# ginevracoal/robustBNNs

Hardware: AMD Instinct MI355X
Metric: attack-samples/sec (test_pts x posterior_samples x PGD_iters) (higher is better)
Workload: dtype f32 (full-width operands as three f16 pieces: 6 exact f16 MFMA product terms per fp32 product, f32 accumulate)

## Files before the change

### include/robustbnns_hip.h

```cpp
#ifndef ROBUSTBNNS_HIP_H
#define ROBUSTBNNS_HIP_H

#include <stddef.h>
#include <stdint.h>

#ifdef __cplusplus
extern "C" {
#endif

#define RBNN_ABI_VERSION 10
#define RBNN_CPAD 16

typedef enum rbnn_status {
    RBNN_OK = 0,
    RBNN_ERR_NULL = -1,
    RBNN_ERR_SHAPE = -2,
    RBNN_ERR_UNSUPPORTED = -3,
    RBNN_ERR_LAUNCH = -4,
    RBNN_ERR_ALIGN = -5
} rbnn_status;

typedef enum rbnn_activation { RBNN_ACT_RELU = 0, RBNN_ACT_LEAKY = 1, RBNN_ACT_SIGM = 2, RBNN_ACT_TANH = 3 } rbnn_activation;
typedef enum rbnn_arch { RBNN_ARCH_FC = 0, RBNN_ARCH_FC2 = 1 } rbnn_arch;

// ... 49 lines not shown
int rbnn_reduce_samples(const float *P, int32_t n_samples, int32_t n_points, int32_t n_classes,
                        float scale, float *out, int32_t ldo, void *stream);

int rbnn_loss_dlogits(int32_t mode, const float *P, const float *Psum, int32_t ldp, const float *G_up,
                      const int32_t *labels, int32_t n_samples, float inv_S, int32_t n_points,
                      int32_t n_classes, float *dZ, void *stream);

int rbnn_fc_input_grad(const rbnn_posterior *net, const int32_t *sample_idx, int32_t n_samples,
                       int32_t n_points, int32_t chunk, const rbnn_workspace *ws,
                       int32_t *n_slabs_out, void *stream);

int rbnn_sum_slabs(const float *slabs, int32_t n_slabs, int32_t n_points, int32_t d_pad, float scale,
                   float *out, int32_t ldo, void *stream);

int rbnn_sum_slabs_norms(const float *slabs, int32_t n_slabs, int32_t n_points, int32_t d_pad, int32_t in_features, float scale,
                         float *out, int32_t ldo, float *linf, float *l2, void *stream);

int rbnn_pgd_alpha(const float *X0, int32_t ldx, int32_t n_points, int32_t in_features,
                   float *alpha, void *stream);

int rbnn_attack_step(float *X, const float *X0, int32_t ldx, const float *G, int32_t n_slabs,
                     size_t slab_stride, int32_t ldg, const float *alpha, float alpha_scalar,
                     float eps, int32_t project, int32_t n_points, int32_t in_features, void *stream);

int rbnn_eval_metrics(const float *out_orig, const float *out_adv, int32_t ldp, const int32_t *labels,
                      int32_t n_points, int32_t n_classes, int32_t *counts, float *rob, void *stream);

int rbnn_pack_rows4(const float *W, int64_t rows, int32_t cols, float *out, void *stream);

typedef struct rbnn_dev_scale {
    uint32_t absmax_bits;
    int32_t  exp;
    float    scale;
    float    inv_scale;
} rbnn_dev_scale;

int rbnn_input_scales(const float *X, int64_t rows, int32_t cols, int32_t ld, float floor_abs, float mul, float add,
                      float cap, rbnn_dev_scale *out, void *stream);

typedef struct rbnn_conv_posterior {
    int32_t activation;
    int32_t hidden;
    int32_t n_classes;
    int32_t n_stored;
    int32_t in_channels;
    int32_t in_width;
// ... 567 lines not shown
```

### robustbnns_amd/_hip.py

```python
import ctypes as C
import os

import torch

from . import _header
from ._header import HipError

_HERE = os.path.dirname(os.path.abspath(__file__))
LIB_PATH = os.path.join(_HERE, "csrc", "librbnn_hip.so")
HEADER_PATH = os.path.join(os.path.dirname(_HERE), "include", "robustbnns_hip.h")

STRUCTS = {
    "Posterior": "rbnn_posterior", "Workspace": "rbnn_workspace", "WorkspaceSizes": "rbnn_workspace_sizes",
    "ConvPosterior": "rbnn_conv_posterior", "ConvWorkspace": "rbnn_conv_workspace", "ConvWorkspaceSizes": "rbnn_conv_workspace_sizes",
    "PieceImages": "rbnn_triple_images", "SplitImages": "rbnn_triple_images", "TripleImages": "rbnn_triple_images",
    "SplitWorkspace": "rbnn_split_workspace", "SplitWorkspaceSizes": "rbnn_split_workspace_sizes",
    "TripleWorkspace": "rbnn_triple_workspace", "TripleWorkspaceSizes": "rbnn_triple_workspace_sizes",
    "SviGuide": "rbnn_svi_guide", "SviFlatTensor": "rbnn_svi_flat_tensor", "SviTrainNet": "rbnn_svi_train_net", "SviTrainWs": "rbnn_svi_train_ws",
    "NnTrainNet": "rbnn_nn_train_net", "NnTrainWs": "rbnn_nn_train_ws",
    "ConvTrainNet": "rbnn_conv_train_net", "ConvTrainWs": "rbnn_conv_train_ws", "ConvTrainBytes": "rbnn_conv_train_bytes",
    "ConvSviTrainNet": "rbnn_conv_svi_train_net",
    "ConvEnsNet": "rbnn_conv_ens_net", "ConvEnsWs": "rbnn_conv_ens_ws", "ConvEnsBytes": "rbnn_conv_ens_bytes",
    "ConvSviLockstepNet": "rbnn_conv_svi_guides_net", "ConvSviLockstepWs": "rbnn_conv_svi_guides_ws", "ConvSviLockstepBytes": "rbnn_conv_svi_guides_bytes",
    "HmcChain": "rbnn_hmc_chain", "HmcLockstep": "rbnn_hmc_lockstep", "ConvHmcChainsNet": "rbnn_conv_hmc_chains_net", "SviLockstep": "rbnn_svi_multi", "SviLockstepAcc": "rbnn_svi_multi_acc",
# ... 117 lines not shown
        check(self.lib.rbnn_loss_dlogits(mode, ptr(P), ptr(Psum), ldp, ptr(G_up), ptr(labels), S, inv_S, N, Cn,
                                         ptr(dZ), stream_of(P)), "rbnn_loss_dlogits")

    def fc_input_grad(self, net, sidx, S, N, chunk, ws):
        w = self._ws(ws)
        n = C.c_int32(0)
        check(self.lib.rbnn_fc_input_grad(C.byref(net.descriptor()), ptr(sidx), S, N, chunk, C.byref(w), C.byref(n),
                                          stream_of(ws["dZ"])), "rbnn_fc_input_grad")
        return n.value

    def sum_slabs(self, slabs, K, N, Dp, scale, out):
        require_gpu(slabs, "slabs")
        check(self.lib.rbnn_sum_slabs(ptr(slabs), K, N, Dp, scale, ptr(out), out.stride(0), stream_of(slabs)), "rbnn_sum_slabs")

    def sum_slabs_norms(self, slabs, K, N, Dp, D, scale, out, linf, l2):
        require_gpu(slabs, "slabs")
        check(self.lib.rbnn_sum_slabs_norms(ptr(slabs), K, N, Dp, D, scale, ptr(out), out.stride(0), ptr(linf), ptr(l2),
                                            stream_of(slabs)), "rbnn_sum_slabs_norms")

    def pgd_alpha(self, X0, D, alpha):
        require_gpu(X0, "X0")
        check(self.lib.rbnn_pgd_alpha(ptr(X0), X0.stride(0), X0.shape[0], D, ptr(alpha), stream_of(X0)), "rbnn_pgd_alpha")

    def attack_step(self, X, X0, G, K, slab_stride, ldg, alpha, alpha_scalar, eps, project, D):
        require_gpu(X, "X")
        check(self.lib.rbnn_attack_step(ptr(X), ptr(X0), X.stride(0), ptr(G), K, slab_stride, ldg, ptr(alpha),
                                        alpha_scalar, eps, int(project), X.shape[0], D, stream_of(X)), "rbnn_attack_step")

    def eval_metrics(self, A, B, labels, Cn, counts, rob):
        require_gpu(A, "outputs")
        check(self.lib.rbnn_eval_metrics(ptr(A), ptr(B), A.stride(0), ptr(labels), A.shape[0], Cn, ptr(counts), ptr(rob),
                                         stream_of(A)), "rbnn_eval_metrics")

    def pack_rows4(self, W, out):
        require_gpu(W, "W")
        cols = W.shape[-1]
        check(self.lib.rbnn_pack_rows4(ptr(W), W.numel() // cols, cols, ptr(out), stream_of(W)), "rbnn_pack_rows4")

    def input_scales(self, X, cols, floor_abs, mul, add, cap, out):
        require_gpu(X, "X")
        check(self.lib.rbnn_input_scales(ptr(X), X.shape[0], cols, X.stride(0), floor_abs, mul, add, cap, ptr(out), stream_of(X)),
              "rbnn_input_scales")
        return out

    def _rows_image(self, name, src, cols, scale_exp, out, ld_dst, dev_scale):
        require_gpu(src, "src")
        ld_src = src.shape[-1]
        check(getattr(self.lib, name)(ptr(src), src.numel() // ld_src, cols, ld_src, scale_exp, ptr(dev_scale), ptr(out), ld_dst, stream_of(src)), name)
# ... 231 lines not shown
```

### robustbnns_amd/csrc/rbnn_kernels.hip

```cpp
#include "rbnn_common.hpp"
#include <stdlib.h>

namespace {

struct FwdArgs {
    const float* X;   long long x_sample_stride;  int ldx;  int N;
    const float* W;   long long w_sample_stride;  int ldw;  int KT;
    const float* b;
    const float* W2;  const float* b2;            int C;    int H;
    const int* sidx;  int S;   int NT;
    float* P;  uint32_t* mask;  float* dact;  float* hid;  int out_kind;
};

template <int ACT, int WH, int HTW, int WN, int NTW, bool LAYER2>
__global__ void __launch_bounds__(64 * WH * WN, (HTW * NTW > 16 ? 2 : (WH * WN) / 2)) fc_forward_kernel(const FwdArgs a) {
    constexpr int BH = WH * HTW * 16, BN = WN * NTW * 16;
    constexpr int TILE = (BH + BN) * 16;
    constexpr bool BITMASK = (ACT == RBNN_ACT_RELU || ACT == RBNN_ACT_LEAKY);
    constexpr int NW = WH * WN;
    static_assert(NW == 4 || NW == 8, "4 or 8 waves per block");
    static_assert(HTW % 2 == 0 && HTW <= 8, "a wave's h range is whole 32-bit mask words, at most 4");
    static_assert(WH * BN * 16 <= 2 * TILE, "the Z^T reduction scratch aliases the tile buffers");
    __shared__ __attribute__((aligned(16))) float lds[2 * TILE];
    float* const zred = lds;
// ... 424 lines not shown
        f32x4 sum = *(const f32x4*)(slabs + off);
        for (int k = 1; k < K; ++k) sum += *(const f32x4*)(slabs + k * slab_stride + off);
        sum = sum * scale;
        *(f32x4*)(out + (long long)n * ldo + c) = sum;
#pragma unroll
        for (int r = 0; r < 4; ++r)
            if (c + r < D) { m = fmaxf(m, fabsf(sum[r])); ss = fmaf(sum[r], sum[r], ss); }
    }
#pragma unroll
    for (int o = 32; o > 0; o >>= 1) { m = fmaxf(m, __shfl_xor(m, o)); ss += __shfl_xor(ss, o); }
    if (lane == 0) { linf[n] = m; l2[n] = sqrtf(ss); }
}

__global__ void pgd_alpha_kernel(const float* __restrict__ X0, int ldx, int N, int D, float* __restrict__ alpha) {
    const int n = blockIdx.x * (blockDim.x >> 6) + (threadIdx.x >> 6), lane = threadIdx.x & 63;
    if (n >= N) return;
    float m = -INFINITY;
    for (int d = lane; d < D; d += 64) m = fmaxf(m, X0[(long long)n * ldx + d]);
#pragma unroll
    for (int o = 32; o > 0; o >>= 1) m = fmaxf(m, __shfl_xor(m, o));
    if (lane == 0) alpha[n] = 2.f / m;
}

__global__ void attack_step_kernel(float* __restrict__ X, const float* __restrict__ X0, int ldx,
                                   const float* __restrict__ G, int K, long long slab_stride, int ldg,
                                   const float* __restrict__ alpha, float alpha_scalar, float eps, int project,
                                   int N, int D) {
    const long long i = (long long)blockIdx.x * blockDim.x + threadIdx.x;
    if (i >= (long long)N * D) return;
    const long long n = i / D;
    const int d = (int)(i % D);
    float g = G[n * ldg + d];
    for (int k = 1; k < K; ++k) g += G[k * slab_stride + n * ldg + d];
    const float sgn = (g > 0.f) ? 1.f : ((g < 0.f) ? -1.f : 0.f);
    const float step = alpha ? alpha[n] : alpha_scalar;
    const float x = X[n * ldx + d];
    float pert = x + step * sgn;
    if (project) {
        const float x0 = X0[n * ldx + d];
        const float eta = fminf(fmaxf(pert - x0, -eps), eps);
        pert = x0 + eta;
    }
    X[n * ldx + d] = fminf(fmaxf(pert, 0.f), 1.f);
}

__global__ void attack_step4_kernel(float* __restrict__ X, const float* __restrict__ X0, int ldx,
                                    const float* __restrict__ G, int K, long long slab_stride, int ldg,
                                    const float* __restrict__ alpha, float alpha_scalar, float eps, int project,
                                    int N, int D4) {
    const long long i = (long long)blockIdx.x * blockDim.x + threadIdx.x;
    if (i >= (long long)N * D4) return;
    const long long n = i / D4;
    const int d = 4 * (int)(i % D4);
    f32x4 g = *(const f32x4*)(G + n * ldg + d);
    for (int k = 1; k < K; ++k) g += *(const f32x4*)(G + k * slab_stride + n * ldg + d);
    const float step = alpha ? alpha[n] : alpha_scalar;
    const f32x4 x = *(const f32x4*)(X + n * ldx + d);
    f32x4 x0 = x, out;
    if (project) x0 = *(const f32x4*)(X0 + n * ldx + d);
#pragma unroll
    for (int r = 0; r < 4; ++r) {
        const float sgn = (g[r] > 0.f) ? 1.f : ((g[r] < 0.f) ? -1.f : 0.f);
        float pert = x[r] + step * sgn;
        if (project) pert = x0[r] + fminf(fmaxf(pert - x0[r], -eps), eps);
        out[r] = fminf(fmaxf(pert, 0.f), 1.f);
    }
    *(f32x4*)(X + n * ldx + d) = out;
}

__global__ void eval_metrics_kernel(const float* __restrict__ A, const float* __restrict__ B, int ldp,
                                    const int* __restrict__ labels, int N, int C, int* __restrict__ counts,
                                    float* __restrict__ rob) {
    const int n = blockIdx.x * blockDim.x + threadIdx.x;
    int ok_a = 0, ok_b = 0;
    if (n < N) {
        float ma = -INFINITY, mb = -INFINITY;
        int ia = 0, ib = 0;
        for (int c = 0; c < C; ++c) {
            const float a = A[(long long)n * ldp + c], b = B[(long long)n * ldp + c];
            if (a > ma) { ma = a; ia = c; }
            if (b > mb) { mb = b; ib = c; }
        }
        float da = 0.f, db = 0.f;
        for (int c = 0; c < C; ++c) { da += expf(A[(long long)n * ldp + c] - ma); db += expf(B[(long long)n * ldp + c] - mb); }
        float diff = 0.f;
        for (int c = 0; c < C; ++c)
            diff = fmaxf(diff, fabsf(expf(A[(long long)n * ldp + c] - ma) / da - expf(B[(long long)n * ldp + c] - mb) / db));
        rob[n] = 1.f - diff;
        ok_a = (ia == labels[n]);
        ok_b = (ib == labels[n]);
// ... 261 lines not shown
    const long long total4 = (long long)N * d_pad / 4;
    hipLaunchKernelGGL(sum_slabs_kernel, dim3((unsigned)((total4 + 255) / 256)), dim3(256), 0, (hipStream_t)stream,
                       slabs, K, (long long)N * d_pad, total4, d_pad / 4, scale, out, ldo);
    return launch_status();
}

int rbnn_sum_slabs_norms(const float* slabs, int32_t K, int32_t N, int32_t d_pad, int32_t D, float scale, float* out, int32_t ldo,
                         float* linf, float* l2, void* stream) {
    if (!slabs || !out || !linf || !l2) return RBNN_ERR_NULL;
    if (K < 1 || N < 1 || d_pad < 4 || (d_pad & 3) || ldo < d_pad || (ldo & 3) || D < 1 || D > d_pad) return RBNN_ERR_SHAPE;
    if (!aligned16(slabs) || !aligned16(out)) return RBNN_ERR_ALIGN;
    hipLaunchKernelGGL(sum_slabs_norms_kernel, dim3((unsigned)((N + 3) / 4)), dim3(256), 0, (hipStream_t)stream,
                       slabs, K, (long long)N * d_pad, N, d_pad, D, scale, out, ldo, linf, l2);
    return launch_status();
}

int rbnn_pgd_alpha(const float* X0, int32_t ldx, int32_t N, int32_t D, float* alpha, void* stream) {
    if (!X0 || !alpha) return RBNN_ERR_NULL;
    if (N < 1 || D < 1 || ldx < D) return RBNN_ERR_SHAPE;
    hipLaunchKernelGGL(pgd_alpha_kernel, dim3((N + 3) / 4), dim3(256), 0, (hipStream_t)stream, X0, ldx, N, D, alpha);
    return launch_status();
}

int rbnn_attack_step(float* X, const float* X0, int32_t ldx, const float* G, int32_t K, size_t slab_stride, int32_t ldg,
                     const float* alpha, float alpha_scalar, float eps, int32_t project, int32_t N, int32_t D, void* stream) {
    if (!X || !G || (project && !X0)) return RBNN_ERR_NULL;
    if (N < 1 || D < 1 || ldx < D || ldg < D || K < 1) return RBNN_ERR_SHAPE;
    if (!(D & 3) && !(ldx & 3) && !(ldg & 3) && !(slab_stride & 3) && aligned16(X) && aligned16(G) && (!project || aligned16(X0))) {
        const long long total4 = (long long)N * (D / 4);
        hipLaunchKernelGGL(attack_step4_kernel, dim3((unsigned)((total4 + 255) / 256)), dim3(256), 0, (hipStream_t)stream,
                           X, X0, ldx, G, K, (long long)slab_stride, ldg, alpha, alpha_scalar, eps, project, N, D / 4);
        return launch_status();
    }
    const long long total = (long long)N * D;
    hipLaunchKernelGGL(attack_step_kernel, dim3((unsigned)((total + 255) / 256)), dim3(256), 0, (hipStream_t)stream,
                       X, X0, ldx, G, K, (long long)slab_stride, ldg, alpha, alpha_scalar, eps, project, N, D);
    return launch_status();
}

int rbnn_eval_metrics(const float* out_orig, const float* out_adv, int32_t ldp, const int32_t* labels, int32_t N, int32_t C,
                      int32_t* counts, float* rob, void* stream) {
    if (!out_orig || !out_adv || !labels || !counts || !rob) return RBNN_ERR_NULL;
    if (N < 1 || C < 1 || ldp < C) return RBNN_ERR_SHAPE;
    if (hipMemsetAsync(counts, 0, 2 * sizeof(int32_t), (hipStream_t)stream) != hipSuccess) return RBNN_ERR_LAUNCH;
    hipLaunchKernelGGL(eval_metrics_kernel, dim3((N + 255) / 256), dim3(256), 0, (hipStream_t)stream,
                       out_orig, out_adv, ldp, labels, N, C, counts, rob);
    return launch_status();
}

int rbnn_pack_rows4(const float* W, int64_t rows, int32_t cols, float* out, void* stream) {
    if (!W || !out) return RBNN_ERR_NULL;
    if (rows < 4 || (rows & 3) || cols < 1) return RBNN_ERR_SHAPE;
    if (!aligned16(out)) return RBNN_ERR_ALIGN;
    const long long total = (rows / 4) * (long long)cols;
    hipLaunchKernelGGL(pack_rows4_kernel, dim3((unsigned)((total + 255) / 256)), dim3(256), 0, (hipStream_t)stream, W, (long long)(rows / 4), cols, out);
    return launch_status();
}

int rbnn_svi_materialize(const float* loc, const float* scale_raw, const float* eps, int64_t n_elem, int32_t S, float* out, void* stream) {
    if (!loc || !scale_raw || !eps || !out) return RBNN_ERR_NULL;
// ... 11 lines not shown
```

### robustbnns_amd/csrc/rbnn_triple.hip

```cpp
#include "rbnn_pieces.hpp"
#include <algorithm>
#include <cstdlib>

namespace {

#ifndef RBNN_X3_PAIR_NOP
#define RBNN_X3_PAIR_NOP 0
#endif
#if RBNN_X3_PAIR_NOP
#define RBNN_X3_PAIR_PAD "\n\ts_nop 1"
#else
#define RBNN_X3_PAIR_PAD ""
#endif
#define RBNN_X3_PAIR_BODY \
    "v_bfe_i32 %[me], %[mw], %[b0], 1\n\t" \
    "v_bfe_i32 %[mo], %[mw], %[b1], 1\n\t" \
    "v_bfi_b32 %[me], %[me], %[cp], %[cn]\n\t" \
    "v_bfi_b32 %[mo], %[mo], %[cp], %[cn]\n\t" \
    "v_fma_mixlo_f16 %[d0], %[ge], %[me], 0\n\t" \
    "v_fma_mixhi_f16 %[d0], %[go], %[mo], 0\n\t" \
    "v_fma_mix_f32 %[re], %[ge], %[me], -%[d0] op_sel_hi:[0,0,1]\n\t" \
    "v_fma_mix_f32 %[ro], %[go], %[mo], -%[d0] op_sel:[0,0,1] op_sel_hi:[0,0,1]\n\t" \
    "v_cvt_pk_f16_f32 %[d1], %[re], %[ro]\n\t" \
    "v_fma_mixlo_f16 %[d2], -%[d1], %[one], %[re] op_sel_hi:[1,0,0]\n\t" \
// ... 510 lines not shown
            for (int k = 0; k < 3; ++k) {
                const f32x4 t = *(const f32x4*)(src + 4 * k);
#pragma unroll
                for (int r = 0; r < 4; ++r) v[4 * k + r] = t[r];
            }
        }
#pragma unroll
        for (int c = 0; c < 10; ++c) pieces_of<3>((n < N && c < C) ? ldexpf(v[c], e) : 0.f, d[c]);
        uint4* const o = dst + ((long long)s * N_pad + n) * 4;
#pragma unroll
        for (int ch = 0; ch < 3; ++ch) {
            union { f16x8 v; uint4 u; } w;
#pragma unroll
            for (int j = 0; j < 8; ++j) w.v[j] = d[j][ch];
            o[ch ^ sw] = w.u;
        }
        union { f16x8 v; uint4 u; } t;
        t.v[0] = d[8][0]; t.v[1] = d[9][0]; t.v[2] = d[8][1]; t.v[3] = d[9][1];
        t.v[4] = d[8][2]; t.v[5] = d[9][2]; t.v[6] = d[8][0]; t.v[7] = d[9][0];
        o[3 ^ sw] = t.u;
    }
}

template <int MODE>
__device__ __forceinline__ void tail_dz(const float* __restrict__ prow, const float (&gmean)[16], int y, int C, float inv_S, float (&out)[16]) {
    float p[16], g[16];
#pragma unroll
    for (int q = 0; q < 4; ++q) {
        const f32x4 v = *(const f32x4*)(prow + 4 * q);
#pragma unroll
        for (int r = 0; r < 4; ++r) p[4 * q + r] = v[r];
    }
    if (MODE == RBNN_LOSS_PER_SAMPLE) {
        ce_softmax_grad<16>(p, C, y, inv_S, g);
    } else {
#pragma unroll
        for (int c = 0; c < 16; ++c) g[c] = gmean[c];
    }
    if (MODE == RBNN_LOSS_MEAN_LOGIT) {
#pragma unroll
        for (int c = 0; c < 16; ++c) out[c] = g[c];
    } else {
        softmax_backward<16>(g, p, C, out);
    }
}

template <int MODE>
__global__ void __launch_bounds__(256) step_tail_x3_kernel(const float* __restrict__ P, const int* __restrict__ labels, int S, float inv_S, int N,
                                                           long long N_pad, int C, float* __restrict__ Psum_out, int ldo,
                                                           uint4* __restrict__ dst, float* __restrict__ gscale) {
    __shared__ float red[16][17];
    __shared__ float psum[16][16];
    const int p = threadIdx.x & 15, q = threadIdx.x >> 4;
    const long long n = (long long)blockIdx.x * 16 + p;
    if (MODE != RBNN_LOSS_PER_SAMPLE) {
        if (q < 4) {
            f32x4 sum = (f32x4){0.f, 0.f, 0.f, 0.f};
            if (n < N)
                for (int s = 0; s < S; ++s) sum += *(const f32x4*)(P + ((long long)s * N + n) * RBNN_CPAD + 4 * q);
#pragma unroll
            for (int r = 0; r < 4; ++r) {
                psum[p][4 * q + r] = sum[r];
                if (Psum_out && n < N && 4 * q + r < C) Psum_out[n * ldo + 4 * q + r] = sum[r];
            }
        }
        __syncthreads();
    }
    const int y = (n < N) ? labels[n] : 0;
    float gmean[16];
    if (MODE != RBNN_LOSS_PER_SAMPLE) {
        float t[16];
#pragma unroll
        for (int c = 0; c < 16; ++c) t[c] = (c < C) ? psum[p][c] * inv_S : 0.f;
        ce_softmax_grad<16>(t, C, y, inv_S, gmean);
    } else {
#pragma unroll
        for (int c = 0; c < 16; ++c) gmean[c] = 0.f;
    }
    float m = 0.f;
    if (n < N)
        for (int s = q; s < S; s += 16) {
            float dz[16];
            tail_dz<MODE>(P + ((long long)s * N + n) * RBNN_CPAD, gmean, y, C, inv_S, dz);
#pragma unroll
            for (int c = 0; c < 12; ++c) if (c < C) m = fmaxf(m, fabsf(dz[c]));
        }
    red[q][p] = m;
    __syncthreads();
    m = 0.f;
#pragma unroll
    for (int i = 0; i < 16; ++i) m = fmaxf(m, red[i][p]);
    int e = 0;
    if (m > 0.f && m < INFINITY) e = min(13 - ilogbf(m), 120);
    if (q == 0) gscale[n] = ldexpf(1.f, -e);
    const int sw = dz_swz3(n);
    for (int s = q; s < S; s += 16) {
        _Float16 d[10][3];
        float dz[16];
#pragma unroll
        for (int c = 0; c < 16; ++c) dz[c] = 0.f;
        if (n < N) tail_dz<MODE>(P + ((long long)s * N + n) * RBNN_CPAD, gmean, y, C, inv_S, dz);
#pragma unroll
        for (int c = 0; c < 10; ++c) pieces_of<3>((n < N && c < C) ? ldexpf(dz[c], e) : 0.f, d[c]);
        uint4* const o = dst + ((long long)s * N_pad + n) * 4;
#pragma unroll
        for (int ch = 0; ch < 3; ++ch) {
            union { f16x8 v; uint4 u; } w;
#pragma unroll
            for (int j = 0; j < 8; ++j) w.v[j] = d[j][ch];
            o[ch ^ sw] = w.u;
        }
        union { f16x8 v; uint4 u; } t;
        t.v[0] = d[8][0]; t.v[1] = d[9][0]; t.v[2] = d[8][1]; t.v[3] = d[9][1];
        t.v[4] = d[8][2]; t.v[5] = d[9][2]; t.v[6] = d[8][0]; t.v[7] = d[9][0];
        o[3 ^ sw] = t.u;
    }
}

__global__ void __launch_bounds__(256) attack_step_x3_kernel(float* __restrict__ X, const float* __restrict__ X0, int ldx, const float* __restrict__ G,
                                                             int K, long long slab_stride, int ldg, const float* __restrict__ alpha, float alpha_scalar,
                                                             float eps, int project, long long N, int D, const rbnn_dev_scale* __restrict__ ds,
                                                             uint4* __restrict__ dst, int groups) {
    const long long i = (long long)blockIdx.x * blockDim.x + threadIdx.x;
    if (i >= N * groups) return;
    const long long n = i / groups;
    const int gq = (int)(i % groups), d0 = 8 * gq;
    const float scale = ds->scale;
    float xn[8];
#pragma unroll
    for (int j = 0; j < 8; ++j) xn[j] = 0.f;
    if (d0 < D) {
        const float step = alpha ? alpha[n] : alpha_scalar;
#pragma unroll
        for (int h = 0; h < 2; ++h) {
            const int d = d0 + 4 * h;
            if (d < D) {
                f32x4 g = *(const f32x4*)(G + n * ldg + d);
                for (int k = 1; k < K; ++k) g += *(const f32x4*)(G + k * slab_stride + n * ldg + d);
// ... 351 lines not shown
int rbnn_fc_forward_triple(const rbnn_posterior* net, const rbnn_triple_images* tp, const rbnn_triple_workspace* tws,
                           int32_t x_exp, const rbnn_dev_scale* dev_scales, int32_t N, const int32_t* sidx, int32_t S,
                           int32_t out_kind, const rbnn_workspace* ws, void* stream) {
    FwdX3Args a = {}, b = {};
    int rc = fc_forward_pieces_args(net, tp, tws ? tws->X_triple : nullptr, tp ? tp->ld_rows : 0, tws ? tws->hid_triple : nullptr, 6, 15,
                                    x_exp, dev_scales, N, sidx, S, out_kind, ws, a, b);
    if (rc) return rc;
    hipStream_t st = (hipStream_t)stream;
    a.x_group_bytes = (unsigned)a.KT * 3072u; a.x_stage_bytes = 3072u;
    if (net->arch != RBNN_ARCH_FC2) return launch_forward_x3<true>(net->activation, a, st);
    if ((rc = launch_forward_x3<false>(net->activation, a, st))) return rc;
    const int NG = (N + 15) / 16;
    b.x_sample_bytes = (long long)NG * 16 * net->hidden * 4; b.x_group_bytes = 2048u; b.x_stage_bytes = (unsigned)NG * 2048u;
    return launch_forward_x3<true, true>(net->activation, b, st);
}

int rbnn_step_tail_triple(int32_t mode, const float* P, const int32_t* labels, int32_t S, float inv_S, int32_t N, int32_t C, float* Psum_out,
                          int32_t ldo, const rbnn_triple_workspace* tws, void* stream) {
    if (!P || !labels || !tws || !tws->dZ_gen || !tws->g_scale) return RBNN_ERR_NULL;
    if (mode != RBNN_LOSS_MEAN_PROB && mode != RBNN_LOSS_PER_SAMPLE && mode != RBNN_LOSS_MEAN_LOGIT) return RBNN_ERR_UNSUPPORTED;
    if (S < 1 || N < 1 || C < 1 || C > 10 || (Psum_out && ldo < C)) return RBNN_ERR_SHAPE;
    if (!aligned16(P) || !aligned16(tws->dZ_gen)) return RBNN_ERR_ALIGN;
    const long long n_pad = mask_ld(N);
    const dim3 grid((unsigned)(n_pad / 16)), block(256);
    hipStream_t st = (hipStream_t)stream;
    if (mode == RBNN_LOSS_MEAN_PROB)
        hipLaunchKernelGGL(step_tail_x3_kernel<RBNN_LOSS_MEAN_PROB>, grid, block, 0, st, P, labels, S, inv_S, N, n_pad, C, Psum_out, ldo, (uint4*)tws->dZ_gen, tws->g_scale);
    else if (mode == RBNN_LOSS_PER_SAMPLE)
        hipLaunchKernelGGL(step_tail_x3_kernel<RBNN_LOSS_PER_SAMPLE>, grid, block, 0, st, P, labels, S, inv_S, N, n_pad, C, Psum_out, ldo, (uint4*)tws->dZ_gen, tws->g_scale);
    else
        hipLaunchKernelGGL(step_tail_x3_kernel<RBNN_LOSS_MEAN_LOGIT>, grid, block, 0, st, P, labels, S, inv_S, N, n_pad, C, Psum_out, ldo, (uint4*)tws->dZ_gen, tws->g_scale);
    return launch_status();
}

int rbnn_attack_step_triple(float* X, const float* X0, int32_t ldx, const float* G, int32_t K, size_t slab_stride, int32_t ldg, const float* alpha,
                            float alpha_scalar, float eps, int32_t project, int32_t N, int32_t D, const rbnn_dev_scale* dev_scale, void* X_triple,
                            int32_t ld_rows, void* stream) {
    if (!X || !G || (project && !X0) || !dev_scale || !X_triple) return RBNN_ERR_NULL;
    if (N < 1 || D < 1 || ldx < D || ldg < D || K < 1 || ld_rows < D || (ld_rows & 31)) return RBNN_ERR_SHAPE;
    if ((D & 3) || (ldx & 3) || (ldg & 3) || (slab_stride & 3)) return RBNN_ERR_SHAPE;
    if (!aligned16(X) || !aligned16(G) || (project && !aligned16(X0)) || !aligned16(X_triple)) return RBNN_ERR_ALIGN;
    const int groups = ld_rows / 8;
    const long long total = (long long)N * groups;
    hipLaunchKernelGGL(attack_step_x3_kernel, dim3((unsigned)((total + 255) / 256)), dim3(256), 0, (hipStream_t)stream,
                       X, X0, ldx, G, K, (long long)slab_stride, ldg, alpha, alpha_scalar, eps, project, (long long)N, D, dev_scale, (uint4*)X_triple, groups);
    return launch_status();
}

int rbnn_fc_input_grad_triple(const rbnn_posterior* net, const rbnn_triple_images* tp, const int32_t* sidx, int32_t S,
                              int32_t N, int32_t chunk, const rbnn_workspace* ws, const rbnn_triple_workspace* tws,
                              int32_t* n_slabs_out, void* stream) {
    return fc_input_grad_pieces(net, tp, sidx, S, N, chunk, ws, tws, n_slabs_out, stream, triple_dz_kernel, true,
                                [](auto mode, int act, const GradPieceArgs& g, hipStream_t st) {
                                    return launch_grad_x3_act<decltype(mode)::value>(act, g, st);
// ... 5 lines not shown
```

### robustbnns_amd/engine.py

```python
import os

import torch

from . import _hip
from ._hip import (LOSS_MEAN_LOGIT, LOSS_MEAN_PROB, LOSS_PER_SAMPLE, LOSS_UPSTREAM, LOSS_UPSTREAM_LOGIT, OUT_LOGITS, OUT_PROBS)

_WS_DTYPE = {"mask1": torch.int32, "mask2": torch.int32}


def to_labels(y, device):
    y = torch.as_tensor(y)
    if y.dim() >= 2:
        y = y.argmax(-1)
    return y.to(device=device, dtype=torch.int32).contiguous()


class _DifferentiableForward(torch.autograd.Function):

    @staticmethod
    def forward(ctx, x, engine, sidx, S, logits):
        ctx.engine, ctx.sidx, ctx.S, ctx.logits = engine, sidx, S, logits
        ctx.save_for_backward(x.detach())
        out = engine.forward_padded(engine.pad_inputs(x), sidx, S, OUT_LOGITS if logits else OUT_PROBS)
        return out[:, :engine.post.C].clone()
# ... 124 lines not shown
    def total_samples(self, S_local):
        if self.world == 1:
            return S_local
        if self._S_total is not None and S_local == self.post.S:
            return self._S_total
        t = torch.tensor([float(S_local)], device=self.device)
        self._allreduce(t)
        return int(round(t.item()))

    def pad_inputs(self, x, clone=False):
        p = self.post
        xf = x.detach().reshape(x.shape[0], -1).to(self.device, torch.float32)
        if xf.shape[1] != p.D:
            raise ValueError(f"inputs flatten to {xf.shape[1]} features, posterior expects {p.D}")
        if p.Dp == p.D:
            xf = xf.contiguous()
            return xf.clone() if (clone or xf.data_ptr() % 16) else xf
        out = torch.zeros(x.shape[0], p.Dp, dtype=torch.float32, device=self.device)
        out[:, :p.D] = xf
        return out

    def unpad(self, Xp, like):
        return Xp[:, :self.post.D].reshape(like.shape).clone()

    def _flat(self, x):
        xf = x.detach().reshape(x.shape[0], -1).to(self.device, torch.float32).contiguous()
        if xf.shape[1] != self.post.D:
            raise ValueError(f"inputs flatten to {xf.shape[1]} features, posterior expects {self.post.D}")
        return xf

    def sample_index(self, n_samples, seeds=None):
        if seeds:
            if len(seeds) != n_samples:
                raise ValueError("Number of seeds should match number of samples.")
        idx = list(range(n_samples)) if seeds is None else [int(s) for s in seeds]
        for i in idx:
            if i >= self.post.S or i < -self.post.S:
                raise IndexError("list index out of range")
        if idx == list(range(self.post.S)):
            return None, len(idx)
        if idx == list(range(len(idx))):
            return None, len(idx)
        t = torch.tensor([i % self.post.S for i in idx], dtype=torch.int32, device=self.device)
        t._rbnn_max_index = max(i % self.post.S for i in idx)
        return t, len(idx)

# ... 251 lines not shown
        N, p = Xp.shape[0], self.post
        G = ws["Gsum"] if "Gsum" in ws else ws["G"]
        if norms is not None and self.world == 1:
            self.k.sum_slabs_norms(ws["slabs"], n_slabs, N, p.Dp, p.D, scale, G, norms[0], norms[1])
            return G
        self.k.sum_slabs(ws["slabs"], n_slabs, N, p.Dp, scale, G)
        self._allreduce(G)
        if norms is not None:
            out = torch.empty_like(G)
            self.k.sum_slabs_norms(G, 1, N, p.Dp, p.D, 1.0, out, norms[0], norms[1])
            return out
        return G

    def loss_gradients(self, x, y, n_samples, seeds=None, norms=False):
        sidx, S = self.sample_index(n_samples, seeds)
        nb = None
        if norms:
            dt = torch.float64 if self.precision == "fp64" else torch.float32
            nb = (torch.empty(x.shape[0], dtype=dt, device=self.device), torch.empty(x.shape[0], dtype=dt, device=self.device))
        xin = self._flat(x) if self.precision == "lowdim" else self.pad_inputs(x)
        G = self.gradient(xin, to_labels(y, self.device), sidx, S, LOSS_PER_SAMPLE, norms=nb)
        return (self.unpad(G, x), nb[0], nb[1]) if norms else self.unpad(G, x)

    def _step(self, X, X0, labels, sidx, S, mode, alpha, alpha_scalar, eps, project):
        p = self.post
        if self.precision == "fp64":
            G = self._fp64_gradient(X, labels, sidx, S, mode)
            return self.k.attack_step_f64(X, X0, G, alpha, alpha_scalar, eps, project, p.D)
        if self.world > 1 and self.pipelined_comm:
            return self._step_sharded(X, X0, labels, sidx, S, mode, alpha, alpha_scalar, eps, project)
        ws, n_slabs, _ = self.gradient_slabs(X, labels, sidx, S, mode)
        if (self.world == 1 and self._carry_image and self._fused_tail(mode, None) and self._scales is not None and "triple" in ws
                and p.D % 4 == 0):
            self.k.attack_step_triple(X, X0, ws["slabs"], n_slabs, X.shape[0] * p.Dp, p.Dp, alpha, alpha_scalar, eps, project, p.D,
                                      self._scales, ws["triple"]["X_triple"], self.post.triple_images().ld_rows)
            ws["x_image_ready"] = X.data_ptr()
        elif self.world == 1:
            self.k.attack_step(X, X0, ws["slabs"], n_slabs, X.shape[0] * p.Dp, p.Dp, alpha, alpha_scalar, eps, project, p.D)
        else:
            G = ws["Gsum"] if "Gsum" in ws else ws["G"]
            self.k.sum_slabs(ws["slabs"], n_slabs, X.shape[0], p.Dp, 1.0, G)
            self._allreduce(G)
            self.k.attack_step(X, X0, G, 1, 0, p.Dp, alpha, alpha_scalar, eps, project, p.D)

    pipelined_comm = True

    def _comm_blocks(self, N, S=None):
        env = os.environ.get("RBNN_COMM_BLOCKS")
        if env is not None:
            want = int(env)
        else:
            want = 2 if (S is not None and S * getattr(self.post, "Hp", 1 << 30) < 16384) else 1
        return max(1, min(want, N // max(1, int(os.environ.get("RBNN_COMM_MIN_POINTS", "512")))))

    def _step_sharded(self, X, X0, labels, sidx, S, mode, alpha, alpha_scalar, eps, project):
        p, N, C = self.post, X.shape[0], self.post.C
        nb = self._comm_blocks(N, S)
        bounds = [0] + [min(N, (N * i // nb + 255) // 256 * 256) for i in range(1, nb)] + [N]
        bounds = sorted(set(bounds))
# ... 9 lines not shown
            h = None
            if need_psum:
                self.k.reduce_samples(ws["P"], S, hi - lo, C, 1.0, ws["Psum"])
                h = self._allreduce_async(ws["Psum"])
            blocks.append((lo, hi, ws, h))
        pending = []
        for lo, hi, ws, h in blocks:
            if h is not None:
                self._wait(h)
            self.k.loss_dlogits(mode, ws["P"], ws["Psum"] if need_psum else None, None, labels[lo:hi], S, inv_S, hi - lo, C, ws["dZ"])
            n_slabs = self._grad_kernels(sidx, S, hi - lo, ws)
            self.k.sum_slabs(ws["slabs"], n_slabs, hi - lo, p.Dp, 1.0, ws["G"])
            pending.append(self._allreduce_async(ws["G"]))
        for (lo, hi, ws, _), h in zip(blocks, pending):
            self._wait(h)
            self.k.attack_step(X[lo:hi], None if X0 is None else X0[lo:hi], ws["G"], 1, 0, p.Dp,
                               None if alpha is None else alpha[lo:hi], alpha_scalar, eps, project, p.D)

    def fgsm(self, x, y, n_samples, epsilon=0.3, seeds=None, mode=LOSS_MEAN_PROB):
        sidx, S = self.sample_index(n_samples, seeds)
        if self.precision == "lowdim":
            out = self._lowdim_attack(self._flat(x), None, to_labels(y, self.device), sidx, S, mode, None, 0.0, False, float(epsilon), False, 1)
            return out.reshape(x.shape)
        X = self.pad_inputs(x, clone=True)
        self._scales = self._input_scales(X, iterates=False)
        try:
            self._step(X, None, to_labels(y, self.device), sidx, S, mode, None, float(epsilon), 0.0, False)
        finally:
            self._scales = None
        return self.unpad(X, x)

    def attack_gradient(self, x, y, n_samples, seeds=None, mode=LOSS_MEAN_PROB):
        sidx, S = self.sample_index(n_samples, seeds)
        xin = self._flat(x) if self.precision == "lowdim" else self.pad_inputs(x)
        return self.gradient(xin, to_labels(y, self.device), sidx, S, mode).clone()

    def fgsm_from_gradient(self, x, G, epsilon):
        p = self.post
        X = self.pad_inputs(x, clone=True)
        if G.dtype == torch.float64:
            self.k.attack_step_f64(X, None, G, None, float(epsilon), 0.0, False, p.D)
            return self.unpad(X, x)
        self.k.attack_step(X, None, G, 1, 0, p.Dp, None, float(epsilon), 0.0, False, p.D)
        return self.unpad(X, x)

    shared_forward = True

    def loss_gradients_and_fgsm(self, x, y, n_samples, epsilon=0.3, seeds=None, mode=LOSS_MEAN_PROB):
        if not self.shared_forward or self.precision in ("lowdim", "fp64") or mode != LOSS_MEAN_PROB:
            return self.loss_gradients(x, y, n_samples, seeds), self.fgsm(x, y, n_samples, epsilon, seeds, mode)
        sidx, S = self.sample_index(n_samples, seeds)
        labels = to_labels(y, self.device)
        p = self.post
        X = self.pad_inputs(x, clone=True)
        N = X.shape[0]
        self._scales = self._input_scales(X, iterates=False)
        try:
            ws = self.workspace(N, S)
            S_tot = self.total_samples(S)
            self._forward_kernels(X, sidx, S, OUT_PROBS, ws)
            G = ws["Gsum"] if "Gsum" in ws else ws["G"]
            n_slabs = self._loss_backward(ws, labels, sidx, S, N, LOSS_PER_SAMPLE, S_tot)
            if self.world == 1:
                self.k.sum_slabs(ws["slabs"], n_slabs, N, p.Dp, 1.0 / S_tot, G)
                expected = self.unpad(G, x)
                n_slabs = self._loss_backward(ws, labels, sidx, S, N, mode, S_tot)
                self.k.attack_step(X, None, ws["slabs"], n_slabs, N * p.Dp, p.Dp, None, float(epsilon), 0.0, False, p.D)
            else:
                G1 = ws.get("G_expected")
                if G1 is None:
                    G1 = ws["G_expected"] = torch.empty_like(G)
                self.k.sum_slabs(ws["slabs"], n_slabs, N, p.Dp, 1.0 / S_tot, G1)
                pending = self._allreduce_async(G1)
                n_slabs = self._loss_backward(ws, labels, sidx, S, N, mode, S_tot)
                self.k.sum_slabs(ws["slabs"], n_slabs, N, p.Dp, 1.0, G)
                self._allreduce(G)
                self.k.attack_step(X, None, G, 1, 0, p.Dp, None, float(epsilon), 0.0, False, p.D)
                self._wait(pending)
                expected = self.unpad(G1, x)
        finally:
            self._scales = None
        return expected, self.unpad(X, x)

    def pgd(self, x, y, n_samples, epsilon, alpha=None, iters=40, seeds=None, mode=LOSS_MEAN_PROB, before_step=None):
        sidx, S = self.sample_index(n_samples, seeds)
        labels = to_labels(y, self.device)
        if self.precision == "lowdim":
            a = 0.0 if alpha is None else float(alpha)
            X0 = self._flat(x)
            if before_step is None:
                return self._lowdim_attack(X0, X0, labels, sidx, S, mode, None, a, alpha is None, float(epsilon), True, iters).reshape(x.shape)
            X = X0
            for it in range(iters):
                if it:
                    before_step()
                X = self._lowdim_attack(X, X0, labels, sidx, S, mode, None, a, alpha is None, float(epsilon), True, 1)
            return X.reshape(x.shape)
        X0 = self.pad_inputs(x, clone=True)
        X = X0.clone()
        alpha_t = None
        if alpha is None:
            alpha_t = torch.empty(X.shape[0], dtype=torch.float32, device=self.device)
            self.k.pgd_alpha(X0, self.post.D, alpha_t)
        self._scales = self._input_scales(X0, iterates=True)
        step = lambda: self._step(X, X0, labels, sidx, S, mode, alpha_t, 0.0 if alpha is None else float(alpha), float(epsilon), True)
# ... 111 lines not shown
```

Baseline: 137.5 million.

## Keep tail-kernel probability rows in registers and add out-of-place FGSM step

The triple-precision step tail kernel is reorganised to handle 4 points per block with 64 sample lanes, each holding up to 4 rows in registers. When S fits (256 or fewer), P is read once instead of up to three times, and dZ is computed once and reused for the scale and for the store. Mean reduction goes through LDS staging and a wave shuffle. Separately, a new out-of-place attack_step entry lets the FGSM paths write into a fresh buffer instead of cloning and padding the input. The cost is higher register pressure in the tail kernel and smaller blocks per point.

```diff
diff --git a/include/robustbnns_hip.h b/include/robustbnns_hip.h
--- a/include/robustbnns_hip.h
+++ b/include/robustbnns_hip.h
@@ -95,6 +95,10 @@
 int rbnn_attack_step(float *X, const float *X0, int32_t ldx, const float *G, int32_t n_slabs,
                      size_t slab_stride, int32_t ldg, const float *alpha, float alpha_scalar,
                      float eps, int32_t project, int32_t n_points, int32_t in_features, void *stream);
+
+int rbnn_attack_step_out(const float *X, const float *X0, int32_t ldx, const float *G, int32_t n_slabs,
+                         size_t slab_stride, int32_t ldg, const float *alpha, float alpha_scalar, float eps,
+                         int32_t project, int32_t n_points, int32_t in_features, float *X_out, void *stream);
 
 int rbnn_eval_metrics(const float *out_orig, const float *out_adv, int32_t ldp, const int32_t *labels,
                       int32_t n_points, int32_t n_classes, int32_t *counts, float *rob, void *stream);
diff --git a/robustbnns_amd/_hip.py b/robustbnns_amd/_hip.py
--- a/robustbnns_amd/_hip.py
+++ b/robustbnns_amd/_hip.py
@@ -163,8 +163,15 @@
         require_gpu(X0, "X0")
         check(self.lib.rbnn_pgd_alpha(ptr(X0), X0.stride(0), X0.shape[0], D, ptr(alpha), stream_of(X0)), "rbnn_pgd_alpha")
 
-    def attack_step(self, X, X0, G, K, slab_stride, ldg, alpha, alpha_scalar, eps, project, D):
-        require_gpu(X, "X")
+    def attack_step(self, X, X0, G, K, slab_stride, ldg, alpha, alpha_scalar, eps, project, D, out=None):
+        require_gpu(X, "X")
+        if out is not None:
+            require_gpu(out, "out")
+            if out.shape != X.shape or out.stride(0) != X.stride(0):
+                raise HipError(f"attack_step: out is {tuple(out.shape)} with row stride {out.stride(0)}, X {tuple(X.shape)} with {X.stride(0)}")
+            check(self.lib.rbnn_attack_step_out(ptr(X), ptr(X0), X.stride(0), ptr(G), K, slab_stride, ldg, ptr(alpha),
+                                                alpha_scalar, eps, int(project), X.shape[0], D, ptr(out), stream_of(X)), "rbnn_attack_step_out")
+            return
         check(self.lib.rbnn_attack_step(ptr(X), ptr(X0), X.stride(0), ptr(G), K, slab_stride, ldg, ptr(alpha),
                                         alpha_scalar, eps, int(project), X.shape[0], D, stream_of(X)), "rbnn_attack_step")
 
diff --git a/robustbnns_amd/csrc/rbnn_kernels.hip b/robustbnns_amd/csrc/rbnn_kernels.hip
--- a/robustbnns_amd/csrc/rbnn_kernels.hip
+++ b/robustbnns_amd/csrc/rbnn_kernels.hip
@@ -470,7 +470,7 @@
     if (lane == 0) alpha[n] = 2.f / m;
 }
 
-__global__ void attack_step_kernel(float* __restrict__ X, const float* __restrict__ X0, int ldx,
+__global__ void attack_step_kernel(const float* X, float* X_out, const float* __restrict__ X0, int ldx,
                                    const float* __restrict__ G, int K, long long slab_stride, int ldg,
                                    const float* __restrict__ alpha, float alpha_scalar, float eps, int project,
                                    int N, int D) {
@@ -489,10 +489,10 @@
         const float eta = fminf(fmaxf(pert - x0, -eps), eps);
         pert = x0 + eta;
     }
-    X[n * ldx + d] = fminf(fmaxf(pert, 0.f), 1.f);
-}
-
-__global__ void attack_step4_kernel(float* __restrict__ X, const float* __restrict__ X0, int ldx,
+    X_out[n * ldx + d] = fminf(fmaxf(pert, 0.f), 1.f);
+}
+
+__global__ void attack_step4_kernel(const float* X, float* X_out, const float* __restrict__ X0, int ldx,
                                     const float* __restrict__ G, int K, long long slab_stride, int ldg,
                                     const float* __restrict__ alpha, float alpha_scalar, float eps, int project,
                                     int N, int D4) {
@@ -513,7 +513,7 @@
         if (project) pert = x0[r] + fminf(fmaxf(pert - x0[r], -eps), eps);
         out[r] = fminf(fmaxf(pert, 0.f), 1.f);
     }
-    *(f32x4*)(X + n * ldx + d) = out;
+    *(f32x4*)(X_out + n * ldx + d) = out;
 }
 
 __global__ void eval_metrics_kernel(const float* __restrict__ A, const float* __restrict__ B, int ldp,
@@ -821,20 +821,35 @@
     return launch_status();
 }
 
+static int attack_step_launch(const float* X, float* X_out, const float* X0, int32_t ldx, const float* G, int32_t K, size_t slab_stride, int32_t ldg,
+                              const float* alpha, float alpha_scalar, float eps, int32_t project, int32_t N, int32_t D, void* stream) {
+    if (!X || !X_out || !G || (project && !X0)) return RBNN_ERR_NULL;
+    if (N < 1 || D < 1 || ldx < D || ldg < D || K < 1) return RBNN_ERR_SHAPE;
+    if (!(D & 3) && !(ldx & 3) && !(ldg & 3) && !(slab_stride & 3) && aligned16(X) && aligned16(X_out) && aligned16(G) && (!project || aligned16(X0))) {
+        const long long total4 = (long long)N * (D / 4);
+        hipLaunchKernelGGL(attack_step4_kernel, dim3((unsigned)((total4 + 255) / 256)), dim3(256), 0, (hipStream_t)stream,
+                           X, X_out, X0, ldx, G, K, (long long)slab_stride, ldg, alpha, alpha_scalar, eps, project, N, D / 4);
+        return launch_status();
+    }
+    const long long total = (long long)N * D;
+    hipLaunchKernelGGL(attack_step_kernel, dim3((unsigned)((total + 255) / 256)), dim3(256), 0, (hipStream_t)stream,
+                       X, X_out, X0, ldx, G, K, (long long)slab_stride, ldg, alpha, alpha_scalar, eps, project, N, D);
+    return launch_status();
+}
+
 int rbnn_attack_step(float* X, const float* X0, int32_t ldx, const float* G, int32_t K, size_t slab_stride, int32_t ldg,
                      const float* alpha, float alpha_scalar, float eps, int32_t project, int32_t N, int32_t D, void* stream) {
-    if (!X || !G || (project && !X0)) return RBNN_ERR_NULL;
-    if (N < 1 || D < 1 || ldx < D || ldg < D || K < 1) return RBNN_ERR_SHAPE;
-    if (!(D & 3) && !(ldx & 3) && !(ldg & 3) && !(slab_stride & 3) && aligned16(X) && aligned16(G) && (!project || aligned16(X0))) {
-        const long long total4 = (long long)N * (D / 4);
-        hipLaunchKernelGGL(attack_step4_kernel, dim3((unsigned)((total4 + 255) / 256)), dim3(256), 0, (hipStream_t)stream,
-                           X, X0, ldx, G, K, (long long)slab_stride, ldg, alpha, alpha_scalar, eps, project, N, D / 4);
-        return launch_status();
-    }
-    const long long total = (long long)N * D;
-    hipLaunchKernelGGL(attack_step_kernel, dim3((unsigned)((total + 255) / 256)), dim3(256), 0, (hipStream_t)stream,
-                       X, X0, ldx, G, K, (long long)slab_stride, ldg, alpha, alpha_scalar, eps, project, N, D);
-    return launch_status();
+    return attack_step_launch(X, X, X0, ldx, G, K, slab_stride, ldg, alpha, alpha_scalar, eps, project, N, D, stream);
+}
+
+int rbnn_attack_step_out(const float* X, const float* X0, int32_t ldx, const float* G, int32_t K, size_t slab_stride, int32_t ldg,
+                         const float* alpha, float alpha_scalar, float eps, int32_t project, int32_t N, int32_t D, float* X_out, void* stream) {
+    if (X && X_out && X != X_out) {
+        const float* const xe = X + ((size_t)N - 1) * (size_t)(ldx > 0 ? ldx : 0) + (D > 0 ? D : 0);
+        const float* const oe = X_out + ((size_t)N - 1) * (size_t)(ldx > 0 ? ldx : 0) + (D > 0 ? D : 0);
+        if (N >= 1 && X < oe && X_out < xe) return RBNN_ERR_SHAPE;
+    }
+    return attack_step_launch(X, X_out, X0, ldx, G, K, slab_stride, ldg, alpha, alpha_scalar, eps, project, N, D, stream);
 }
 
 int rbnn_eval_metrics(const float* out_orig, const float* out_adv, int32_t ldp, const int32_t* labels, int32_t N, int32_t C,
diff --git a/robustbnns_amd/csrc/rbnn_triple.hip b/robustbnns_amd/csrc/rbnn_triple.hip
--- a/robustbnns_amd/csrc/rbnn_triple.hip
+++ b/robustbnns_amd/csrc/rbnn_triple.hip
@@ -556,15 +556,12 @@
     }
 }
 
+constexpr int TAIL_PTS = 4, TAIL_QL = 64, TAIL_KEEP = 4;
+constexpr int TAIL_S_RESIDENT = TAIL_QL * TAIL_KEEP;
+
 template <int MODE>
-__device__ __forceinline__ void tail_dz(const float* __restrict__ prow, const float (&gmean)[16], int y, int C, float inv_S, float (&out)[16]) {
-    float p[16], g[16];
-#pragma unroll
-    for (int q = 0; q < 4; ++q) {
-        const f32x4 v = *(const f32x4*)(prow + 4 * q);
-#pragma unroll
-        for (int r = 0; r < 4; ++r) p[4 * q + r] = v[r];
-    }
+__device__ __forceinline__ void tail_dz(const float (&p)[16], const float (&gmean)[16], int y, int C, float inv_S, float (&out)[16]) {
+    float g[16];
     if (MODE == RBNN_LOSS_PER_SAMPLE) {
         ce_softmax_grad<16>(p, C, y, inv_S, g);
     } else {
@@ -579,28 +576,83 @@
     }
 }
 
-template <int MODE>
+__device__ __forceinline__ void tail_store(const float (&dz)[16], bool live, int C, int e, uint4* __restrict__ o, int sw) {
+    _Float16 d[10][3];
+#pragma unroll
+    for (int c = 0; c < 10; ++c) pieces_of<3>((live && c < C) ? ldexpf(dz[c], e) : 0.f, d[c]);
+#pragma unroll
+    for (int ch = 0; ch < 3; ++ch) {
+        union { f16x8 v; uint4 u; } w;
+#pragma unroll
+        for (int j = 0; j < 8; ++j) w.v[j] = d[j][ch];
+        o[ch ^ sw] = w.u;
+    }
+    union { f16x8 v; uint4 u; } t;
+    t.v[0] = d[8][0]; t.v[1] = d[9][0]; t.v[2] = d[8][1]; t.v[3] = d[9][1];
+    t.v[4] = d[8][2]; t.v[5] = d[9][2]; t.v[6] = d[8][0]; t.v[7] = d[9][0];
+    o[3 ^ sw] = t.u;
+}
+
+template <int MODE, bool RESIDENT>
 __global__ void __launch_bounds__(256) step_tail_x3_kernel(const float* __restrict__ P, const int* __restrict__ labels, int S, float inv_S, int N,
                                                            long long N_pad, int C, float* __restrict__ Psum_out, int ldo,
                                                            uint4* __restrict__ dst, float* __restrict__ gscale) {
-    __shared__ float red[16][17];
-    __shared__ float psum[16][16];
-    const int p = threadIdx.x & 15, q = threadIdx.x >> 4;
-    const long long n = (long long)blockIdx.x * 16 + p;
+    __shared__ f32x4 stage[TAIL_QL][TAIL_PTS][4];
+    __shared__ float psum[TAIL_PTS][16];
+    __shared__ float red[4][TAIL_PTS];
+    const int tid = threadIdx.x, p = tid & (TAIL_PTS - 1), q = tid / TAIL_PTS;
+    const long long n = (long long)blockIdx.x * TAIL_PTS + p;
+    const bool live = n < N;
+    float rows[TAIL_KEEP][16];
+    auto load_rows = [&](int s0) {
+#pragma unroll
+        for (int i = 0; i < TAIL_KEEP; ++i) {
+            const int s = s0 + i * TAIL_QL + q;
+            const bool on = live && s < S;
+            const float* const src = P + ((long long)(on ? s : 0) * N + (on ? n : 0)) * RBNN_CPAD;
+#pragma unroll
+            for (int k = 0; k < 4; ++k) {
+                f32x4 v = (f32x4){0.f, 0.f, 0.f, 0.f};
+                if (on) v = *(const f32x4*)(src + 4 * k);
+#pragma unroll
+                for (int r = 0; r < 4; ++r) rows[i][4 * k + r] = v[r];
+            }
+        }
+    };
+    const int S_trips = RESIDENT ? 1 : S;
+    if (RESIDENT) load_rows(0);
     if (MODE != RBNN_LOSS_PER_SAMPLE) {
-        if (q < 4) {
-            f32x4 sum = (f32x4){0.f, 0.f, 0.f, 0.f};
-            if (n < N)
-                for (int s = 0; s < S; ++s) sum += *(const f32x4*)(P + ((long long)s * N + n) * RBNN_CPAD + 4 * q);
+        const int sp = tid & (TAIL_PTS - 1), cq = (tid / TAIL_PTS) & 3;
+        f32x4 sum = (f32x4){0.f, 0.f, 0.f, 0.f};
+        for (int s0 = 0; s0 < S_trips; s0 += TAIL_S_RESIDENT) {
+            if (!RESIDENT) load_rows(s0);
+#pragma unroll
+            for (int i = 0; i < TAIL_KEEP; ++i) {
+                const int base = s0 + i * TAIL_QL;
+                if (base < S) {
+#pragma unroll
+                    for (int k = 0; k < 4; ++k) stage[q][p][k] = (f32x4){rows[i][4 * k], rows[i][4 * k + 1], rows[i][4 * k + 2], rows[i][4 * k + 3]};
+                    __syncthreads();
+                    if (tid < 4 * TAIL_PTS) {
+                        const int cnt = min(TAIL_QL, S - base);
+#pragma unroll 8
+                        for (int j = 0; j < cnt; ++j) sum += stage[j][sp][cq];
+                    }
+                    __syncthreads();
+                }
+            }
+        }
+        if (tid < 4 * TAIL_PTS) {
+            const long long ns = (long long)blockIdx.x * TAIL_PTS + sp;
 #pragma unroll
             for (int r = 0; r < 4; ++r) {
-                psum[p][4 * q + r] = sum[r];
-                if (Psum_out && n < N && 4 * q + r < C) Psum_out[n * ldo + 4 * q + r] = sum[r];
+                psum[sp][4 * cq + r] = sum[r];
+                if (Psum_out && ns < N && 4 * cq + r < C) Psum_out[ns * ldo + 4 * cq + r] = sum[r];
             }
         }
         __syncthreads();
     }
-    const int y = (n < N) ? labels[n] : 0;
+    const int y = live ? labels[n] : 0;
     float gmean[16];
     if (MODE != RBNN_LOSS_PER_SAMPLE) {
         float t[16];
@@ -612,42 +664,43 @@
         for (int c = 0; c < 16; ++c) gmean[c] = 0.f;
     }
     float m = 0.f;
-    if (n < N)
-        for (int s = q; s < S; s += 16) {
-            float dz[16];
-            tail_dz<MODE>(P + ((long long)s * N + n) * RBNN_CPAD, gmean, y, C, inv_S, dz);
-#pragma unroll
-            for (int c = 0; c < 12; ++c) if (c < C) m = fmaxf(m, fabsf(dz[c]));
-        }
-    red[q][p] = m;
+    float dzk[TAIL_KEEP][16];
+    for (int s0 = 0; s0 < S_trips; s0 += TAIL_S_RESIDENT) {
+        if (!RESIDENT) load_rows(s0);
+#pragma unroll
+        for (int i = 0; i < TAIL_KEEP; ++i) {
+#pragma unroll
+            for (int c = 0; c < 16; ++c) dzk[i][c] = 0.f;
+            if (live && s0 + i * TAIL_QL + q < S) {
+                tail_dz<MODE>(rows[i], gmean, y, C, inv_S, dzk[i]);
+#pragma unroll
+                for (int c = 0; c < 12; ++c) if (c < C) m = fmaxf(m, fabsf(dzk[i][c]));
+            }
+        }
+    }
+#pragma unroll
+    for (int o = TAIL_PTS; o < 64; o <<= 1) m = fmaxf(m, __shfl_xor(m, o));
+    if ((tid & 63) < TAIL_PTS) red[tid >> 6][p] = m;
     __syncthreads();
-    m = 0.f;
-#pragma unroll
-    for (int i = 0; i < 16; ++i) m = fmaxf(m, red[i][p]);
+    m = fmaxf(fmaxf(red[0][p], red[1][p]), fmaxf(red[2][p], red[3][p]));
     int e = 0;
     if (m > 0.f && m < INFINITY) e = min(13 - ilogbf(m), 120);
     if (q == 0) gscale[n] = ldexpf(1.f, -e);
     const int sw = dz_swz3(n);
-    for (int s = q; s < S; s += 16) {
-        _Float16 d[10][3];
-        float dz[16];
-#pragma unroll
-        for (int c = 0; c < 16; ++c) dz[c] = 0.f;
-        if (n < N) tail_dz<MODE>(P + ((long long)s * N + n) * RBNN_CPAD, gmean, y, C, inv_S, dz);
-#pragma unroll
-        for (int c = 0; c < 10; ++c) pieces_of<3>((n < N && c < C) ? ldexpf(dz[c], e) : 0.f, d[c]);
-        uint4* const o = dst + ((long long)s * N_pad + n) * 4;
-#pragma unroll
-        for (int ch = 0; ch < 3; ++ch) {
-            union { f16x8 v; uint4 u; } w;
-#pragma unroll
-            for (int j = 0; j < 8; ++j) w.v[j] = d[j][ch];
-            o[ch ^ sw] = w.u;
-        }
-        union { f16x8 v; uint4 u; } t;
-        t.v[0] = d[8][0]; t.v[1] = d[9][0]; t.v[2] = d[8][1]; t.v[3] = d[9][1];
-        t.v[4] = d[8][2]; t.v[5] = d[9][2]; t.v[6] = d[8][0]; t.v[7] = d[9][0];
-        o[3 ^ sw] = t.u;
+    for (int s0 = 0; s0 < S_trips; s0 += TAIL_S_RESIDENT) {
+        if (!RESIDENT) load_rows(s0);
+#pragma unroll
+        for (int i = 0; i < TAIL_KEEP; ++i) {
+            const int s = s0 + i * TAIL_QL + q;
+            if (s < S) {
+                if (!RESIDENT) {
+#pragma unroll
+                    for (int c = 0; c < 16; ++c) dzk[i][c] = 0.f;
+                    if (live) tail_dz<MODE>(rows[i], gmean, y, C, inv_S, dzk[i]);
+                }
+                tail_store(dzk[i], live, C, e, dst + ((long long)s * N_pad + n) * 4, sw);
+            }
+        }
     }
 }
 
@@ -1045,14 +1098,16 @@
     if (S < 1 || N < 1 || C < 1 || C > 10 || (Psum_out && ldo < C)) return RBNN_ERR_SHAPE;
     if (!aligned16(P) || !aligned16(tws->dZ_gen)) return RBNN_ERR_ALIGN;
     const long long n_pad = mask_ld(N);
-    const dim3 grid((unsigned)(n_pad / 16)), block(256);
+    const dim3 grid((unsigned)(n_pad / TAIL_PTS)), block(TAIL_PTS * TAIL_QL);
     hipStream_t st = (hipStream_t)stream;
+    auto launch = [&](auto kernel) { hipLaunchKernelGGL(kernel, grid, block, 0, st, P, labels, S, inv_S, N, n_pad, C, Psum_out, ldo, (uint4*)tws->dZ_gen, tws->g_scale); };
+    const bool resident = S <= TAIL_S_RESIDENT;
     if (mode == RBNN_LOSS_MEAN_PROB)
-        hipLaunchKernelGGL(step_tail_x3_kernel<RBNN_LOSS_MEAN_PROB>, grid, block, 0, st, P, labels, S, inv_S, N, n_pad, C, Psum_out, ldo, (uint4*)tws->dZ_gen, tws->g_scale);
+        resident ? launch(step_tail_x3_kernel<RBNN_LOSS_MEAN_PROB, true>) : launch(step_tail_x3_kernel<RBNN_LOSS_MEAN_PROB, false>);
     else if (mode == RBNN_LOSS_PER_SAMPLE)
-        hipLaunchKernelGGL(step_tail_x3_kernel<RBNN_LOSS_PER_SAMPLE>, grid, block, 0, st, P, labels, S, inv_S, N, n_pad, C, Psum_out, ldo, (uint4*)tws->dZ_gen, tws->g_scale);
+        resident ? launch(step_tail_x3_kernel<RBNN_LOSS_PER_SAMPLE, true>) : launch(step_tail_x3_kernel<RBNN_LOSS_PER_SAMPLE, false>);
     else
-        hipLaunchKernelGGL(step_tail_x3_kernel<RBNN_LOSS_MEAN_LOGIT>, grid, block, 0, st, P, labels, S, inv_S, N, n_pad, C, Psum_out, ldo, (uint4*)tws->dZ_gen, tws->g_scale);
+        resident ? launch(step_tail_x3_kernel<RBNN_LOSS_MEAN_LOGIT, true>) : launch(step_tail_x3_kernel<RBNN_LOSS_MEAN_LOGIT, false>);
     return launch_status();
 }
 
diff --git a/robustbnns_amd/engine.py b/robustbnns_amd/engine.py
--- a/robustbnns_amd/engine.py
+++ b/robustbnns_amd/engine.py
@@ -170,6 +170,15 @@
 
     def unpad(self, Xp, like):
         return Xp[:, :self.post.D].reshape(like.shape).clone()
+
+    def _fgsm_buffers(self, x):
+        p = self.post
+        if (isinstance(self.k, _hip.HipKernels) and self.world == 1 and self.precision != "fp64" and p.Dp == p.D and torch.is_tensor(x)
+                and x.dtype == torch.float32 and x.is_contiguous() and x.data_ptr() % 16 == 0):
+            X = self.pad_inputs(x)
+            if X.data_ptr() == x.data_ptr():
+                return X, torch.empty_like(X)
+        return self.pad_inputs(x, clone=True), None
 
     def _flat(self, x):
         xf = x.detach().reshape(x.shape[0], -1).to(self.device, torch.float32).contiguous()
@@ -467,8 +476,9 @@
         G = self.gradient(xin, to_labels(y, self.device), sidx, S, LOSS_PER_SAMPLE, norms=nb)
         return (self.unpad(G, x), nb[0], nb[1]) if norms else self.unpad(G, x)
 
-    def _step(self, X, X0, labels, sidx, S, mode, alpha, alpha_scalar, eps, project):
+    def _step(self, X, X0, labels, sidx, S, mode, alpha, alpha_scalar, eps, project, out=None):
         p = self.post
+        assert out is None or (self.world == 1 and self.precision != "fp64" and not self._carry_image)
         if self.precision == "fp64":
             G = self._fp64_gradient(X, labels, sidx, S, mode)
             return self.k.attack_step_f64(X, X0, G, alpha, alpha_scalar, eps, project, p.D)
@@ -480,6 +490,8 @@
             self.k.attack_step_triple(X, X0, ws["slabs"], n_slabs, X.shape[0] * p.Dp, p.Dp, alpha, alpha_scalar, eps, project, p.D,
                                       self._scales, ws["triple"]["X_triple"], self.post.triple_images().ld_rows)
             ws["x_image_ready"] = X.data_ptr()
+        elif self.world == 1 and out is not None:
+            self.k.attack_step(X, X0, ws["slabs"], n_slabs, X.shape[0] * p.Dp, p.Dp, alpha, alpha_scalar, eps, project, p.D, out=out)
         elif self.world == 1:
             self.k.attack_step(X, X0, ws["slabs"], n_slabs, X.shape[0] * p.Dp, p.Dp, alpha, alpha_scalar, eps, project, p.D)
         else:
@@ -535,13 +547,13 @@
         if self.precision == "lowdim":
             out = self._lowdim_attack(self._flat(x), None, to_labels(y, self.device), sidx, S, mode, None, 0.0, False, float(epsilon), False, 1)
             return out.reshape(x.shape)
-        X = self.pad_inputs(x, clone=True)
+        X, out = self._fgsm_buffers(x)
         self._scales = self._input_scales(X, iterates=False)
         try:
-            self._step(X, None, to_labels(y, self.device), sidx, S, mode, None, float(epsilon), 0.0, False)
+            self._step(X, None, to_labels(y, self.device), sidx, S, mode, None, float(epsilon), 0.0, False, out=out)
         finally:
             self._scales = None
-        return self.unpad(X, x)
+        return self.unpad(X, x) if out is None else out.reshape(x.shape)
 
     def attack_gradient(self, x, y, n_samples, seeds=None, mode=LOSS_MEAN_PROB):
         sidx, S = self.sample_index(n_samples, seeds)
@@ -550,10 +562,14 @@
 
     def fgsm_from_gradient(self, x, G, epsilon):
         p = self.post
-        X = self.pad_inputs(x, clone=True)
         if G.dtype == torch.float64:
+            X = self.pad_inputs(x, clone=True)
             self.k.attack_step_f64(X, None, G, None, float(epsilon), 0.0, False, p.D)
             return self.unpad(X, x)
+        X, out = self._fgsm_buffers(x)
+        if out is not None:
+            self.k.attack_step(X, None, G, 1, 0, p.Dp, None, float(epsilon), 0.0, False, p.D, out=out)
+            return out.reshape(x.shape)
         self.k.attack_step(X, None, G, 1, 0, p.Dp, None, float(epsilon), 0.0, False, p.D)
         return self.unpad(X, x)
 
@@ -565,7 +581,7 @@
         sidx, S = self.sample_index(n_samples, seeds)
         labels = to_labels(y, self.device)
         p = self.post
-        X = self.pad_inputs(x, clone=True)
+        X, out = self._fgsm_buffers(x)
         N = X.shape[0]
         self._scales = self._input_scales(X, iterates=False)
         try:
@@ -578,7 +594,10 @@
                 self.k.sum_slabs(ws["slabs"], n_slabs, N, p.Dp, 1.0 / S_tot, G)
                 expected = self.unpad(G, x)
                 n_slabs = self._loss_backward(ws, labels, sidx, S, N, mode, S_tot)
-                self.k.attack_step(X, None, ws["slabs"], n_slabs, N * p.Dp, p.Dp, None, float(epsilon), 0.0, False, p.D)
+                if out is not None:
+                    self.k.attack_step(X, None, ws["slabs"], n_slabs, N * p.Dp, p.Dp, None, float(epsilon), 0.0, False, p.D, out=out)
+                else:
+                    self.k.attack_step(X, None, ws["slabs"], n_slabs, N * p.Dp, p.Dp, None, float(epsilon), 0.0, False, p.D)
             else:
                 G1 = ws.get("G_expected")
                 if G1 is None:
@@ -593,7 +612,7 @@
                 expected = self.unpad(G1, x)
         finally:
             self._scales = None
-        return expected, self.unpad(X, x)
+        return expected, (self.unpad(X, x) if out is None else out.reshape(x.shape))
 
     def pgd(self, x, y, n_samples, epsilon, alpha=None, iters=40, seeds=None, mode=LOSS_MEAN_PROB, before_step=None):
         sidx, S = self.sample_index(n_samples, seeds)
```

New measurement: 139.2 million (median of 6 runs). 1.01x the previous value.
